# chronoxor/CppServer

Measured on AMD Instinct MI355X. Metric: WS payload mask/unmask GiB/s (device-resident), batched 64KiB frames, higher is better.
Workload: dtype u8; 1 GPU; C2 unmask-only: 4096 masked binary frames x 65536 B payload, one key per frame; parallelism=independent batch per GPU (dp1), frames=4096, payload_bytes_per_frame=65536, wire_bytes=268492800

## Files before the change

cppserver_amd/csrc/wsg_kernels.hip:

```cpp
#include "wsg_device.h"

namespace wsg {

namespace {

typedef uint64_t v4u64 __attribute__((ext_vector_type(4)));

constexpr int MAXF = 4;

#ifndef WSG_ENC_NT_SRC
#define WSG_ENC_NT_SRC 0
#endif
#ifndef WSG_ENC_NT_HI
#define WSG_ENC_NT_HI 1
#endif
#ifndef WSG_DIAG_ENC
#define WSG_DIAG_ENC 0
#endif
#ifndef WSG_DIAG
#define WSG_DIAG 0
#endif
#ifndef WSG_DIAG_FAN
#define WSG_DIAG_FAN 0
#endif
#ifndef WSG_DIAG_NOINFO
#define WSG_DIAG_NOINFO 0
#endif
#ifndef WSG_DEC_WAVES
#define WSG_DEC_WAVES 1
#endif
#ifndef WSG_DEC_RELOAD
#define WSG_DEC_RELOAD 1
#endif
#ifndef WSG_FAN_PERIOD
#define WSG_FAN_PERIOD 1
#endif
#ifndef WSG_FAN_UNROLL
#define WSG_FAN_UNROLL 1
#endif
#ifndef WSG_FAN_CAP
#define WSG_FAN_CAP 0
#endif
#ifndef WSG_FAN_MANY_WPC
#define WSG_FAN_MANY_WPC 46
#endif
#ifndef WSG_FAN_MANY_WPB
#define WSG_FAN_MANY_WPB 0
#endif
#ifndef WSG_FAN_KV
#define WSG_FAN_KV 2
#endif

__device__ __forceinline__ v4u ld16_sys(const void* p)
{
    v4u r;
    asm volatile("global_load_dwordx4 %0, %1, off sc0 sc1\n\ts_waitcnt vmcnt(0)" : "=v"(r) : "v"(p) : "memory");
    return r;
}

#ifndef WSG_OUT_SC1
#define WSG_OUT_SC1 0
#endif
#ifndef WSG_OUT_AUX
#define WSG_OUT_AUX 16
#endif
#ifndef WSG_ENC_SC1
#define WSG_ENC_SC1 0
#endif
#ifndef WSG_FAN_SC1
#define WSG_FAN_SC1 1
#endif
struct OutTile {
    uint8_t* p;
    bool sc1;
    __amdgpu_buffer_rsrc_t rs;
    __device__ __forceinline__ OutTile(uint8_t* base, uint32_t bytes, bool write_through = WSG_OUT_SC1 != 0)
        : p(base), sc1(write_through)
    {
        if (sc1)
            rs = __builtin_amdgcn_make_buffer_rsrc(base, 0, bytes, 0x00020000);
    }
    __device__ __forceinline__ void put(uint32_t o, v4u v) const
    {
        if (sc1)
            __builtin_amdgcn_raw_buffer_store_b128(v, rs, o, 0, WSG_OUT_AUX);
        else
            st16nt(p + o, v);
    }
};

#ifndef WSG_STAGE_FPL
#define WSG_STAGE_FPL 2
#endif
constexpr int SPL = WSG_STAGE_FPL;
constexpr int LDSF = BLOCK * SPL;

__device__ __forceinline__ void fill_tiles_wave(uint32_t* tile_first, uint64_t lo, uint64_t hi, uint32_t frame)
{
    const uint32_t lane = threadIdx.x & 63;
    constexpr uint64_t kShort = 16;
    if (hi > lo && hi - lo <= kShort)
        for (uint64_t t = lo; t < hi; ++t)
            tile_first[t] = frame;
    uint64_t pending = __ballot(hi > lo + kShort);
    while (pending) {
        const int j = __builtin_ctzll(pending);
        pending &= pending - 1;
        const uint64_t a = lane_bcast(lo, j), b = lane_bcast(hi, j);
        const uint32_t fj = __builtin_amdgcn_readlane(frame, j);
        for (uint64_t t = a + lane; t < b; t += 64)
            tile_first[t] = fj;
    }
}

__device__ __forceinline__ uint64_t lane_off(int u) { return (uint64_t(u) * BLOCK + threadIdx.x) * CHUNK; }

}


namespace {

__device__ __forceinline__ uint64_t fs_at(const uint64_t* __restrict__ fs, uint32_t n, int64_t i)
{
    return fs[min<int64_t>(i, int64_t(n) - 1)];
}

__device__ __forceinline__ int64_t search8(const uint64_t* __restrict__ fs, uint32_t a, uint32_t b, uint64_t p)
{
    while (a < b) {
        const uint32_t step = (b - a + 8) / 9;
        uint64_t v[8];
#pragma unroll
        for (int k = 0; k < 8; ++k)
            v[k] = fs[min(a - 1 + step * (k + 1), b - 1)];
        uint32_t na = a, nb = b;
#pragma unroll
        for (int k = 0; k < 8; ++k) {
            const uint32_t ix = min(a - 1 + step * (k + 1), b - 1);
            if (ix >= na && ix < nb) {
                if (v[k] <= p)
                    na = ix + 1;
                else
                    nb = ix;
            }
        }
        a = na;
        b = nb;
    }
    return int64_t(a) - 1;
}

struct TileLoc {
    int64_t f0;
    uint32_t first;
    uint64_t st[MAXF + 1];
};

__device__ __forceinline__ uint64_t tile_guess(uint32_t n, double frames_per_byte, uint64_t base)
{
    return uni(min(uint64_t(double(base) * frames_per_byte), uint64_t(n - 1)));
}

__device__ __forceinline__ uint32_t probe_index(uint64_t g, uint32_t stride, uint32_t n, int k)
{
    const int64_t i = int64_t(g) + int64_t(k - 32) * int64_t(stride);
    return uint32_t(max<int64_t>(0, min<int64_t>(i, int64_t(n) - 1)));
}

__device__ __forceinline__ void locate(const uint64_t* __restrict__ fs, uint32_t n, uint64_t g, uint32_t stride,
                                       uint64_t probe, uint64_t base, TileLoc& L)
{
    uint64_t w[MAXF + 2];
#pragma unroll
    for (int k = 0; k < MAXF + 2; ++k) {
        const uint64_t x = fs_at(fs, n, int64_t(g) + k);
        w[k] = (g + k < n) ? x : ~uint64_t(0);
    }
    if (w[0] <= base && base < w[1]) {
        L.f0 = int64_t(g);
        L.first = uint32_t(g);
#pragma unroll
        for (int k = 0; k <= MAXF; ++k)
            L.st[k] = w[k];
        return;
    }
    const uint64_t below = __ballot(probe <= base);
    const int m = __builtin_popcountll(below);
    uint32_t a = m > 0 ? probe_index(g, stride, n, m - 1) + 1 : 0;
    uint32_t b = m < 64 ? probe_index(g, stride, n, m) : n;
    if (m == 0 && probe_index(g, stride, n, 0) == 0)
        b = 0;
    L.f0 = search8(fs, a, b, base);
    L.first = uint32_t(L.f0 < 0 ? 0 : L.f0);
#pragma unroll
    for (int k = 0; k <= MAXF; ++k) {
        const uint64_t x = fs_at(fs, n, int64_t(L.first) + k);
        L.st[k] = (uint64_t(L.first) + k < n) ? x : ~uint64_t(0);
    }
}

struct Seg {
    uint32_t lo, hi, kr;
};

__device__ __forceinline__ Seg tile_seg(uint64_t po, uint64_t pe, uint32_t key, uint64_t base, uint32_t span)
{
    Seg s;
    s.lo = po <= base ? 0u : uint32_t(min<uint64_t>(po - base, span));
    s.hi = pe <= base ? 0u : uint32_t(min<uint64_t>(pe - base, span));
    if (s.hi < s.lo)
        s.hi = s.lo;
    s.kr = key_rot(key, uint32_t(base - po));
    return s;
}

__device__ __forceinline__ v4u seg_xor(uint32_t o, const Seg& s)
{
    if (s.hi <= o || s.lo >= o + CHUNK)
        return v4u{0, 0, 0, 0};
    const int a = s.lo > o ? int(s.lo - o) : 0;
    const int b = s.hi < o + CHUNK ? int(s.hi - o) : int(CHUNK);
    v4u m;
#pragma unroll
    for (int d = 0; d < 4; ++d)
        m[d] = s.kr & low_bytes(b - 4 * d) & ~low_bytes(a - 4 * d);
    return m;
}

struct TileIn {
    uint64_t base, g, probe;
    v4u v[UNROLL];
};

__device__ __forceinline__ void load_tile(TileIn& T, const uint8_t* __restrict__ wire, uint64_t wire_len,
                                          const uint64_t* __restrict__ fs, uint32_t n, double frames_per_byte,
                                          uint32_t stride, uint64_t base)
{
    T.base = base;
    T.g = tile_guess(n, frames_per_byte, base);
#if WSG_DIAG == 7
    T.probe = 0;
#else
    T.probe = fs[probe_index(T.g, stride, n, int(threadIdx.x & 63))];
#endif
    __builtin_amdgcn_sched_barrier(0);
    const uint64_t last_blk = (wire_len - 1) & ~uint64_t(CHUNK - 1);
#pragma unroll
    for (int u = 0; u < UNROLL; ++u)
        T.v[u] = ld16nt(wire + min(base + lane_off(u), last_blk));
}

__device__ __forceinline__ void process_tile(const TileIn& T, const uint8_t* __restrict__ wire, uint8_t* out,
                                             uint64_t wire_len, const uint64_t* __restrict__ fs, uint32_t n,
                                             uint32_t stride)
{
    const uint64_t base = T.base;
    const uint64_t tend = min(base + TILE, wire_len);
    const uint32_t span = uint32_t(tend - base);
    const bool full = span == TILE;
    const uint64_t g = T.g;
    const uint64_t probe = T.probe;
    const v4u* v = T.v;
    auto keep_probe = [&]() {
        if (n == 0 && probe == ~uint64_t(0))
            out[0] = 0;
    };
    TileLoc L;
    locate(fs, n, g, stride, probe, base, L);
    int c = 0;
#pragma unroll
    for (int k = 0; k <= MAXF; ++k) {
        const bool touches = uint64_t(L.first) + k < n && (k == 0 ? L.f0 >= 0 || L.st[0] < tend : L.st[k] < tend);
        if (touches && c == k)
            c = k + 1;
    }

    if (WSG_DIAG == 5 || (full && c <= MAXF)) {
        Seg S[MAXF];
#pragma unroll
        for (int k = 0; k < MAXF; ++k) {
            S[k] = Seg{0, 0, 0};
            if (k < c) {
                wsg_recv_info r;
                const uint64_t lim = (uint64_t(L.first) + k + 1 < n) ? L.st[k + 1] : wire_len;
                frame_parse(wire, wire_len, L.st[k], lim, r);
                const Seg g = tile_seg(r.payload_off, r.payload_off + r.len, r.key, base, span);
                S[k] = Seg{uni(g.lo), uni(g.hi), uni(g.kr)};
            }
        }
#if WSG_DIAG == 5
        if (true) {
#else
        if (S[0].lo == 0 && S[0].hi == TILE) {
#endif
            const OutTile ot(out + base, uint32_t(TILE));
#pragma unroll
            for (int u = 0; u < UNROLL; ++u)
                ot.put(uint32_t(lane_off(u)), v[u] ^ S[0].kr);
            keep_probe();
            return;
        }
        const OutTile ot(out + base, uint32_t(TILE));
#pragma unroll
        for (int u = 0; u < UNROLL; ++u) {
            const uint32_t o = uint32_t(lane_off(u));
            uint32_t kx = 0;
            bool cut = false;
#pragma unroll
            for (int k = 0; k < MAXF; ++k) {
                kx = (S[k].lo <= o && o + CHUNK <= S[k].hi) ? S[k].kr : kx;
                cut |= (S[k].lo > o && S[k].lo < o + CHUNK) || (S[k].hi > o && S[k].hi < o + CHUNK);
            }
            v4u x = v4u{kx, kx, kx, kx};
            if (cut) {
                x = seg_xor(o, S[0]);
#pragma unroll
                for (int k = 1; k < MAXF; ++k)
                    x |= seg_xor(o, S[k]);
            }
            ot.put(o, v[u] ^ x);
        }
        keep_probe();
        return;
    }

    __shared__ uint32_t s_lo[LDSF], s_hi[LDSF], s_kr[LDSF];
    __shared__ uint32_t s_wcnt[BLOCK / 64];
    auto stage = [&](uint64_t r0, int& cnt, bool& more) {
        uint64_t sj[SPL], lim[SPL];
        bool touch[SPL];
#pragma unroll
        for (int q = 0; q < SPL; ++q) {
            const uint64_t fi = r0 + uint64_t(q) * BLOCK + threadIdx.x;
            sj[q] = ~uint64_t(0);
            lim[q] = wire_len;
            if (fi < n) {
                sj[q] = fs[fi];
                lim[q] = fi + 1 < n ? fs[fi + 1] : wire_len;
            }
            touch[q] = fi < n && (fi == L.first || sj[q] < tend);
        }
        uint32_t wc = 0;
#pragma unroll
        for (int q = 0; q < SPL; ++q)
            wc += uint32_t(__builtin_popcountll(__ballot(touch[q])));
        const bool last_more = __ballot(threadIdx.x == BLOCK - 1 && touch[SPL - 1] &&
                                        r0 + uint64_t(LDSF) < n && lim[SPL - 1] < tend) != 0;
        __syncthreads();
        if ((threadIdx.x & 63) == 0)
            s_wcnt[threadIdx.x >> 6] = wc | (last_more ? 0x80000000u : 0u);
        __syncthreads();
        cnt = 0;
        more = false;
#pragma unroll
        for (int w = 0; w < BLOCK / 64; ++w) {
            const uint32_t x = s_wcnt[w];
            cnt += int(x & 0x7FFFFFFFu);
            more = more || (x >> 31) != 0;
        }
#pragma unroll 1
        for (int q = 0; q < SPL; ++q) {
            const int slot = q * BLOCK + int(threadIdx.x);
            if (slot < cnt) {
                wsg_recv_info r;
                frame_parse(wire, wire_len, sj[q], lim[q], r);
                const Seg g = tile_seg(r.payload_off, r.payload_off + r.len, r.key, base, span);
                s_lo[slot] = g.lo;
                s_hi[slot] = g.hi;
                s_kr[slot] = g.kr;
            }
        }
        __syncthreads();
    };
    auto chunk_xor = [&](uint32_t o, int cnt) {
        int lo = 0, hi = cnt;
#pragma unroll 1
        while (lo < hi) {
            const int mid = (lo + hi) >> 1;
            if (s_hi[mid] <= o)
                lo = mid + 1;
            else
                hi = mid;
        }
        v4u x = {0, 0, 0, 0};
#pragma unroll 1
        for (int j = lo; j < cnt && s_lo[j] < o + CHUNK; ++j)
            x |= seg_xor(o, Seg{s_lo[j], s_hi[j], s_kr[j]});
        return x;
    };
    __shared__ v4u s_acc[UNROLL][BLOCK];
#pragma unroll 1
    for (uint64_t r0 = L.first;; r0 += LDSF) {
        int cnt;
        bool more;
        stage(r0, cnt, more);
#pragma unroll 1
        for (int u = 0; u < UNROLL; ++u) {
            const v4u x = chunk_xor(uint32_t(lane_off(u)), cnt);
            s_acc[u][threadIdx.x] = (r0 == L.first) ? x : (s_acc[u][threadIdx.x] | x);
        }
        if (!more)
            break;
    }
    {
        const OutTile ot(out + base, uint32_t(TILE));
#pragma unroll 1
        for (int u = 0; u < UNROLL; ++u) {
            const uint32_t o = uint32_t(lane_off(u));
            if (o + CHUNK <= span) {
                ot.put(o, ld16(wire + base + o) ^ s_acc[u][threadIdx.x]);
            } else if (o < span) {
                uint8_t* b = reinterpret_cast<uint8_t*>(&s_acc[u][threadIdx.x]);
#pragma unroll 1
                for (uint32_t k = 0; k < span - o; ++k)
                    out[base + o + k] = uint8_t(wire[base + o + k] ^ b[k]);
            }
        }
    }
    keep_probe();
}

}

__global__ __launch_bounds__(BLOCK) __attribute__((amdgpu_waves_per_eu(WSG_DEC_WAVES))) void k_decode(const uint8_t* __restrict__ wire, uint8_t* out, uint64_t wire_len,
                                                  const uint64_t* __restrict__ fs, uint32_t n, double frames_per_byte,
                                                  uint32_t stride, wsg_recv_info* __restrict__ info,
                                                  unsigned long long* err, uint64_t num_tiles)
{
    {
        const uint64_t fstride = uint64_t(gridDim.x) * BLOCK;
        for (uint64_t i0 = uint64_t(blockIdx.x) * BLOCK + (threadIdx.x & ~63u); i0 < n && !WSG_DIAG_NOINFO;
             i0 += fstride) {
            const uint64_t i = i0 + (threadIdx.x & 63u);
            if (i < n) {
                wsg_recv_info r;
                const int e = frame_parse(wire, wire_len, fs[i], i + 1 < n ? fs[i + 1] : wire_len, r);
                if (e != 0)
                    latch(err, i, e);
                store_info(info + i, r);
            }
        }
    }

#if WSG_DIAG == 6
    for (uint64_t t = blockIdx.x; t < num_tiles; t += gridDim.x) {
        const uint64_t base = t * TILE;
        if (base + TILE > wire_len)
            break;
        v4u v[UNROLL];
#pragma unroll
        for (int u = 0; u < UNROLL; ++u) {
            v[u] = ld16nt(wire + base + lane_off(u));
#ifdef WSG_DIAG_ORD
            __builtin_amdgcn_sched_barrier(0);
#endif
        }
#pragma unroll
        for (int u = 0; u < UNROLL; ++u)
            st16nt(out + base + lane_off(u), v[u] ^ 0x9u);
    }
    return;
#endif
    for (uint64_t t = blockIdx.x; t < num_tiles; t += gridDim.x) {
        TileIn a;
        load_tile(a, wire, wire_len, fs, n, frames_per_byte, stride, t * TILE);
        process_tile(a, wire, out, wire_len, fs, n, stride);
    }
}


namespace {

struct Desc {
    uint64_t src_off, len;
    uint32_t key;
    int32_t status;
    uint8_t opcode;
    bool mask;
};

__device__ __forceinline__ Desc load_desc(const wsg_send_desc* d)
{
    const uint32_t* w = reinterpret_cast<const uint32_t*>(d);
    Desc r;
    r.src_off = uint64_t(w[0]) | (uint64_t(w[1]) << 32);
    r.len = uint64_t(w[2]) | (uint64_t(w[3]) << 32);
    r.key = w[4];
    r.status = int32_t(w[5]);
    r.opcode = uint8_t(w[6]);
    r.mask = ((w[6] >> 8) & 0xFFu) != 0;
    return r;
}
static_assert(offsetof(wsg_send_desc, key) == 16 && offsetof(wsg_send_desc, opcode) == 24 &&
                  offsetof(wsg_send_desc, mask) == 25,
              "wsg_send_desc layout");

struct StagedBlocks {
    const v4u* s;
    const uint8_t* base;
    __device__ v4u operator()(const uint8_t* p) const { return s[(p - base) >> 4]; }
};

__device__ __forceinline__ v4u shr_bytes(v4u x, uint64_t o)
{
    return o >= CHUNK ? v4u{0, 0, 0, 0} : funnel(x, v4u{0, 0, 0, 0}, uint32_t(o));
}
__device__ __forceinline__ v4u shl_bytes(v4u x, uint64_t s)
{
    return s == 0 ? x : s >= CHUNK ? v4u{0, 0, 0, 0} : funnel(v4u{0, 0, 0, 0}, x, uint32_t(CHUNK - s));
}
__device__ __forceinline__ v4u low_bytes(uint64_t n)
{
    const uint64_t lo = n >= 8 ? ~uint64_t(0) : (uint64_t(1) << (8 * n)) - 1;
    const uint64_t hi = n >= 16 ? ~uint64_t(0) : n <= 8 ? 0 : (uint64_t(1) << (8 * (n - 8))) - 1;
    return v4u{uint32_t(lo), uint32_t(lo >> 32), uint32_t(hi), uint32_t(hi >> 32)};
}

__device__ __forceinline__ void edge_chunk2(const FrameRec& R, v4u head, uint64_t p, uint8_t* __restrict__ wire)
{
    if (p + CHUNK <= R.off)
        return;
    v4u w = p >= R.off ? shr_bytes(head, p - R.off) : shl_bytes(head, R.off - p);
    const int64_t data_len = int64_t(R.end - R.data_w);
    const int64_t rel = int64_t(p) - int64_t(R.data_w);
    if (rel < data_len && rel + int64_t(CHUNK) > 0) {
        const v4u d = fan_window(R.src, uint64_t(data_len), rel);
        const uint32_t kw = key_rot(R.key, uint32_t(p - R.pw));
        const uint64_t lo = p < R.data_w ? R.data_w - p : 0;
        const uint64_t hi = R.end - p < CHUNK ? R.end - p : CHUNK;
        w |= (d ^ v4u{kw, kw, kw, kw}) & (low_bytes(hi) & ~low_bytes(lo));
    }
    const uint32_t o_lo = p < R.off ? uint32_t(R.off - p) : 0u;
    const uint32_t o_hi = R.end - p < CHUNK ? uint32_t(R.end - p) : uint32_t(CHUNK);
    if ((o_lo == 0 && o_hi == CHUNK) || (WSG_DIAG_ENC & 4)) {
        st16nt(wire + p, w);
        return;
    }
    uint32_t* w32 = reinterpret_cast<uint32_t*>(wire + p);
#pragma unroll
    for (uint32_t k = 0; k < 4; ++k) {
        const uint32_t b0 = 4 * k, b1 = b0 + 4;
        if (b0 >= o_lo && b1 <= o_hi) {
            w32[k] = w[k];
        } else {
            for (uint32_t j = max(b0, o_lo); j < min(b1, o_hi); ++j)
                wire[p + j] = uint8_t(w[k] >> (8 * (j - b0)));
        }
    }
}

template <bool NT>
struct Piece {
    FrameRec R;
    uint64_t lo = 0, hi = 0;
    uint32_t s = 0;
    uint32_t kw = 0;
    bool live = false;
    uint32_t dmask = 0;
    v4u a[EU], b[EU];

    __device__ __forceinline__ void load(const FrameRec& rec, uint64_t k, bool exists)
    {
        R = rec;
        const uint32_t lane = threadIdx.x & 63;
        lo = (R.off & ~(PIECE_ALIGN - 1)) + k * PIECE;
        live = exists && lo < R.end;
        hi = min(lo + PIECE, R.end);
        s = (WSG_DIAG_ENC & 2) ? 0u
                                : uint32_t((reinterpret_cast<uintptr_t>(R.src) + (lo - R.data_w)) & 15u);
        kw = key_rot(R.key, uint32_t(lo - R.pw));
#pragma unroll
        for (int u = 0; u < EU; ++u) {
            const uint64_t p = lo + (uint64_t(u) * 64 + lane) * CHUNK;
            const bool d = live && p < hi && p >= R.data_w && p + CHUNK <= R.end;
            dmask |= uint32_t(d) << u;
            const uint8_t* a0 = R.src + (int64_t(p - R.data_w) - int64_t(s));
            a[u] = d ? (NT ? ld16nt(a0) : ld16(a0)) : v4u{0, 0, 0, 0};
        }
#pragma unroll
        for (int u = 0; u < EU; ++u) {
            const uint64_t p = lo + (uint64_t(u) * 64 + lane) * CHUNK;
            const uint8_t* a0 = R.src + (int64_t(p - R.data_w) - int64_t(s));
            b[u] = ((dmask >> u) & 1u) && s ? ((NT && WSG_ENC_NT_HI) ? ld16nt(a0 + CHUNK) : ld16(a0 + CHUNK))
                                          : v4u{0, 0, 0, 0};
        }
    }

    __device__ __forceinline__ void store(uint8_t* __restrict__ wire) const
    {
        if (!live)
            return;
        const uint32_t lane = threadIdx.x & 63;
        const OutTile ot(wire + lo, uint32_t(PIECE), WSG_ENC_SC1 != 0);
        v4u head = {0, 0, 0, 0};
        if (lo < R.data_w)
            head = frame_head(R);
#pragma unroll
        for (int u = 0; u < EU; ++u) {
            const uint64_t p = lo + (uint64_t(u) * 64 + lane) * CHUNK;
            if ((dmask >> u) & 1u) {
                ot.put(uint32_t(p - lo), (s ? funnel(a[u], b[u], s) : a[u]) ^ kw);
            } else if (p < hi && !(WSG_DIAG_ENC & 1)) {
                edge_chunk2(R, head, p, wire);
            }
        }
    }
};

__device__ __forceinline__ uint64_t pieces_of(uint64_t frame_bytes)
{
    return (frame_bytes + PIECE_ALIGN - 1 + PIECE - 1) / PIECE;
}

}

template <bool PIECES>
__global__ __launch_bounds__(BLOCK) void k_encode_scan_local(const wsg_send_desc* __restrict__ desc, uint32_t n,
                                                             uint64_t* __restrict__ wire_off,
                                                             uint32_t* __restrict__ piece_start,
                                                             uint64_t* __restrict__ block_sums,
                                                             uint64_t* __restrict__ block_psums)
{
    const uint64_t first = uint64_t(blockIdx.x) * SCAN_ITEMS;
    uint64_t sz[SCAN_PER_LANE];
#pragma unroll
    for (int k = 0; k < SCAN_PER_LANE; ++k) {
        const uint64_t i = first + uint64_t(k) * BLOCK + threadIdx.x;
        sz[k] = 0;
        if (i < n) {
            const Desc d = load_desc(desc + i);
            const SendGeom g = send_geom(d.opcode, d.mask, d.len, d.status);
            sz[k] = g.hdr + g.body;
        }
    }
    uint64_t run = 0, run_p = 0;
#pragma unroll
    for (int k = 0; k < SCAN_PER_LANE; ++k) {
        const uint64_t i = first + uint64_t(k) * BLOCK + threadIdx.x;
        uint64_t tot, tot_p = 0;
        const uint64_t ex = block_scan_ex(sz[k], OpAdd{}, &tot);
        uint64_t ex_p = 0;
        if (PIECES)
            ex_p = block_scan_ex(sz[k] ? pieces_of(sz[k]) : 0, OpAdd{}, &tot_p);
        if (i < n) {
            wire_off[i] = run + ex;
            if (PIECES)
                piece_start[i] = uint32_t(run_p + ex_p);
        }
        run += tot;
        run_p += tot_p;
    }
    if (threadIdx.x == 0) {
        block_sums[blockIdx.x] = run;
        if (PIECES)
            block_psums[blockIdx.x] = run_p;
    }
}

__global__ __launch_bounds__(BLOCK) void k_encode_scan_blocks(const uint64_t* __restrict__ block_sums,
                                                              const uint64_t* __restrict__ block_psums, uint32_t nb,
                                                              uint64_t* __restrict__ block_prefix,
                                                              uint64_t* __restrict__ block_pprefix,
                                                              uint64_t* __restrict__ wire_off,
                                                              uint32_t* __restrict__ piece_start, uint32_t n)
{
    const uint64_t carry = scan_partials(block_sums, block_prefix, nb, OpAdd{});
    const uint64_t carry_p = scan_partials(block_psums, block_pprefix, nb, OpAdd{});
    if (threadIdx.x == 0) {
        wire_off[n] = carry;
        piece_start[n] = uint32_t(carry_p);
    }
}

__global__ __launch_bounds__(BLOCK) void k_encode_finalize(const wsg_send_desc* __restrict__ desc, uint32_t n,
                                                           uint64_t* __restrict__ wire_off,
                                                           uint32_t* __restrict__ piece_start,
                                                           const uint64_t* __restrict__ block_prefix,
                                                           const uint64_t* __restrict__ block_pprefix,
                                                           uint32_t* __restrict__ piece_frame, uint64_t pieces_cap,
                                                           uint64_t wire_cap, unsigned long long* err)
{
    if (blockIdx.x * BLOCK + (threadIdx.x & ~63u) >= n)
        return;
    const uint32_t i = blockIdx.x * BLOCK + threadIdx.x;
    uint64_t lo = 0, hi = 0;
    if (i < n) {
        const wsg_send_desc d = desc[i];
        const SendGeom g = send_geom(d.opcode, d.mask != 0, d.len, d.status);
        const uint64_t off = wire_off[i] + block_prefix[i / SCAN_ITEMS];
        const uint64_t ps = piece_start[i] + block_pprefix[i / SCAN_ITEMS];
        const uint64_t end = off + g.hdr + g.body;
        wire_off[i] = off;
        piece_start[i] = uint32_t(ps);
        if (end > wire_cap)
            latch(err, i, WSG_ENOMEM);
        piece_range(ps, ps + pieces_of(g.hdr + g.body), pieces_cap, lo, hi);
    }
    fill_tiles_wave(piece_frame, lo, hi, i);
}

__global__ __launch_bounds__(BLOCK) void k_encode_mask(const uint8_t* __restrict__ payload,
                                                       const wsg_send_desc* __restrict__ desc, uint32_t n,
                                                       const uint64_t* __restrict__ wire_off,
                                                       const uint32_t* __restrict__ piece_start,
                                                       const uint32_t* __restrict__ piece_frame,
                                                       uint8_t* __restrict__ wire, uint64_t wire_cap,
                                                       uint32_t q_begin, uint32_t q_end)
{
    const uint32_t waves = gridDim.x * (BLOCK / 64);
    uint32_t q = q_begin + blockIdx.x * (BLOCK / 64) + wave_id();
    if (wire_off[n] > wire_cap)
        return;
    const uint32_t pieces = min(piece_start[n], q_end);
    struct Meta {
        Desc d;
        uint64_t off;
        uint32_t ps;
    };
// ... 1003 lines not shown
```

Baseline: 2956 GiB/s.

## Keep tile payload in LDS, parse headers from it, batch searches

The decode slow path now seeds the LDS accumulator with the tile's already-loaded wire data and XORs masks into it in place. This removes the second global read of the wire at store time. Frame headers that fall inside the tile are parsed from LDS through a block accessor instead of global memory, and frame-start loads for the next round are issued before the current round's work. The per-chunk binary searches are merged into one branchless lockstep search across all unrolled chunks. The cost is more LDS traffic and more register use for the prefetched starts.

```diff
diff --git a/cppserver_amd/csrc/wsg_kernels.hip b/cppserver_amd/csrc/wsg_kernels.hip
--- a/cppserver_amd/csrc/wsg_kernels.hip
+++ b/cppserver_amd/csrc/wsg_kernels.hip
@@ -28,9 +28,6 @@
 #endif
 #ifndef WSG_DEC_WAVES
 #define WSG_DEC_WAVES 1
-#endif
-#ifndef WSG_DEC_RELOAD
-#define WSG_DEC_RELOAD 1
 #endif
 #ifndef WSG_FAN_PERIOD
 #define WSG_FAN_PERIOD 1
@@ -326,18 +323,28 @@
 
     __shared__ uint32_t s_lo[LDSF], s_hi[LDSF], s_kr[LDSF];
     __shared__ uint32_t s_wcnt[BLOCK / 64];
-    auto stage = [&](uint64_t r0, int& cnt, bool& more) {
-        uint64_t sj[SPL], lim[SPL];
-        bool touch[SPL];
+    __shared__ v4u s_acc[UNROLL][BLOCK];
+    static_assert(sizeof(s_acc) == TILE, "s_acc is one tile: chunk o / CHUNK of the tile is slot o / CHUNK");
+    auto starts = [&](uint64_t r0, uint64_t (&sj)[SPL], uint64_t (&lim)[SPL]) {
 #pragma unroll
         for (int q = 0; q < SPL; ++q) {
             const uint64_t fi = r0 + uint64_t(q) * BLOCK + threadIdx.x;
-            sj[q] = ~uint64_t(0);
-            lim[q] = wire_len;
-            if (fi < n) {
-                sj[q] = fs[fi];
-                lim[q] = fi + 1 < n ? fs[fi + 1] : wire_len;
-            }
+            const uint64_t a = fs_at(fs, n, int64_t(fi)), b = fs_at(fs, n, int64_t(fi + 1));
+            sj[q] = fi < n ? a : ~uint64_t(0);
+            lim[q] = fi + 1 < n ? b : wire_len;
+        }
+    };
+    auto tile_block = [&](uint64_t a) -> v4u {
+        const uint64_t d = a - base;
+        if (d < TILE)
+            return (&s_acc[0][0])[uint32_t(d) / CHUNK];
+        return ld16(wire + a);
+    };
+    auto stage = [&](uint64_t r0, const uint64_t (&sj)[SPL], const uint64_t (&lim)[SPL], int& cnt, bool& more) {
+        bool touch[SPL];
+#pragma unroll
+        for (int q = 0; q < SPL; ++q) {
+            const uint64_t fi = r0 + uint64_t(q) * BLOCK + threadIdx.x;
             touch[q] = fi < n && (fi == L.first || sj[q] < tend);
         }
         uint32_t wc = 0;
@@ -363,7 +370,7 @@
             const int slot = q * BLOCK + int(threadIdx.x);
             if (slot < cnt) {
                 wsg_recv_info r;
-                frame_parse(wire, wire_len, sj[q], lim[q], r);
+                frame_parse_b(tile_block, wire_len, sj[q], lim[q], r);
                 const Seg g = tile_seg(r.payload_off, r.payload_off + r.len, r.key, base, span);
                 s_lo[slot] = g.lo;
                 s_hi[slot] = g.hi;
@@ -372,35 +379,46 @@
         }
         __syncthreads();
     };
-    auto chunk_xor = [&](uint32_t o, int cnt) {
-        int lo = 0, hi = cnt;
+    auto round_xor = [&](int cnt) {
+        uint32_t pos[UNROLL];
+#pragma unroll
+        for (int u = 0; u < UNROLL; ++u)
+            pos[u] = 0;
 #pragma unroll 1
-        while (lo < hi) {
-            const int mid = (lo + hi) >> 1;
-            if (s_hi[mid] <= o)
-                lo = mid + 1;
-            else
-                hi = mid;
-        }
-        v4u x = {0, 0, 0, 0};
+        for (uint32_t step = cnt > 0 ? 1u << (31 - __builtin_clz(uint32_t(cnt))) : 0u; step; step >>= 1) {
+#pragma unroll
+            for (int u = 0; u < UNROLL; ++u) {
+                const uint32_t p = pos[u] + step;
+                const uint32_t e = s_hi[min(p, uint32_t(LDSF)) - 1];
+                if (p <= uint32_t(cnt) && e <= uint32_t(lane_off(u)))
+                    pos[u] = p;
+            }
+        }
+#pragma unroll
+        for (int u = 0; u < UNROLL; ++u) {
+            const uint32_t o = uint32_t(lane_off(u));
+            v4u x = {0, 0, 0, 0};
 #pragma unroll 1
-        for (int j = lo; j < cnt && s_lo[j] < o + CHUNK; ++j)
-            x |= seg_xor(o, Seg{s_lo[j], s_hi[j], s_kr[j]});
-        return x;
+            for (int j = int(pos[u]); j < cnt && s_lo[j] < o + CHUNK; ++j)
+                x |= seg_xor(o, Seg{s_lo[j], s_hi[j], s_kr[j]});
+            s_acc[u][threadIdx.x] ^= x;
+        }
     };
-    __shared__ v4u s_acc[UNROLL][BLOCK];
+    uint64_t sj[SPL], lim[SPL];
+    starts(L.first, sj, lim);
+#pragma unroll
+    for (int u = 0; u < UNROLL; ++u)
+        s_acc[u][threadIdx.x] = v[u];
 #pragma unroll 1
-    for (uint64_t r0 = L.first;; r0 += LDSF) {
+    for (uint64_t r0 = L.first;;) {
         int cnt;
         bool more;
-        stage(r0, cnt, more);
-#pragma unroll 1
-        for (int u = 0; u < UNROLL; ++u) {
-            const v4u x = chunk_xor(uint32_t(lane_off(u)), cnt);
-            s_acc[u][threadIdx.x] = (r0 == L.first) ? x : (s_acc[u][threadIdx.x] | x);
-        }
+        stage(r0, sj, lim, cnt, more);
+        round_xor(cnt);
         if (!more)
             break;
+        r0 += LDSF;
+        starts(r0, sj, lim);
     }
     {
         const OutTile ot(out + base, uint32_t(TILE));
@@ -408,12 +426,12 @@
         for (int u = 0; u < UNROLL; ++u) {
             const uint32_t o = uint32_t(lane_off(u));
             if (o + CHUNK <= span) {
-                ot.put(o, ld16(wire + base + o) ^ s_acc[u][threadIdx.x]);
+                ot.put(o, s_acc[u][threadIdx.x]);
             } else if (o < span) {
-                uint8_t* b = reinterpret_cast<uint8_t*>(&s_acc[u][threadIdx.x]);
+                const uint8_t* b = reinterpret_cast<const uint8_t*>(&s_acc[u][threadIdx.x]);
 #pragma unroll 1
                 for (uint32_t k = 0; k < span - o; ++k)
-                    out[base + o + k] = uint8_t(wire[base + o + k] ^ b[k]);
+                    out[base + o + k] = b[k];
             }
         }
     }
```

Measured after the change: 2952 GiB/s (median of 2 runs). Within noise of the previous version (-0.2%).
